# jagannatharjun/AntiZ

Measured on AMD Instinct MI355X. Metric: input MB/s precompressed (1 GB synthetic, 100k streams) at 1/2/4/8 MI355X, higher is better.
Workload: dtype u8

## Files before the change

antiz_amd/csrc/k_deflate.hip:

```cpp
#include <hip/hip_runtime.h>
#include "atz_device.h"

#define LDS __attribute__((address_space(3)))
#define CONSTANT __attribute__((address_space(4)))
#define GLOBAL __attribute__((address_space(1)))

#ifndef ATZ_VISITED_CHECK
#define ATZ_VISITED_CHECK 1
#endif
#ifndef ATZ_VISITED_MAX
#define ATZ_VISITED_MAX 8
#endif
#ifndef ATZ_NOSLIDE_PATH
#define ATZ_NOSLIDE_PATH 1
#endif
#ifndef ATZ_STEP_SPLIT
#define ATZ_STEP_SPLIT 0
#endif
#ifndef ATZ_STEP_CLOCKS
#define ATZ_STEP_CLOCKS 0
#endif
#if ATZ_STEP_CLOCKS
#define STEP_CLOCK() clock64()
#else
// ... 572 lines not shown
    o.x = (bf > 2 ? (bf << 23) | (df << 8) : 0u) | s0;
    if (jb.fast) o.y = ((p - reach) << 16) | (budget_out << 12) | (slot << 1) | valid;
    else o.y = (bq > 2 ? (bq << 23) | (dq << 8) : 0u) | valid;
    r[p] = o;
  }
}

__global__ __launch_bounds__(256) void k_match(const uint8_t* __restrict__ infl, const uint32_t* __restrict__ chains,
                                              uint2* __restrict__ R, const MatchJob* __restrict__ jobs) {
  const MatchJob jb = jobs[blockIdx.x];
  const uint8_t* in = infl + jb.infl_off;
  match_positions(jb, in, reinterpret_cast<const uint32_t*>(in), chains, R);
}

static constexpr uint32_t PREV_NIL = 0xffffu;
#ifndef ATZ_MATCH_THREADS
#define ATZ_MATCH_THREADS 1024
#endif
static constexpr uint32_t MATCH_THREADS = ATZ_MATCH_THREADS;
struct LdsWin {
  const LDS uint32_t* p;
  uint32_t off;
  __device__ __forceinline__ uint32_t operator[](uint32_t w) const { return p[w - off]; }
};
__global__ __launch_bounds__(MATCH_THREADS) void k_match_lds(const uint8_t* __restrict__ infl, const uint32_t* __restrict__ chains,
                                                  uint2* __restrict__ R, const MatchJob* __restrict__ jobs) {
  extern __shared__ uint32_t dyn_lds[];
  const MatchJob jb = jobs[blockIdx.x];
  const uint8_t* in = infl + jb.infl_off;
  const uint32_t* g32 = reinterpret_cast<const uint32_t*>(in);
  const uint32_t n = (uint32_t)jb.n, npad = (n + 63) & ~63u;
  const uint32_t* sidx = chains + jb.chain_off;
  const uint32_t* bpos = sidx + npad;
  const uint32_t maxdist = (1u << jb.window) - 262;
  const uint32_t lo = (uint32_t)jb.p0 > maxdist ? ((uint32_t)jb.p0 - maxdist) & ~3u : 0u;
  const uint32_t w0 = lo >> 2;
  const uint64_t want = jb.p1 + 258 + 24;
  const uint32_t nw = (uint32_t)(((want < n ? want : n) + 3) >> 2) - w0;
  LDS uint32_t* l32 = (LDS uint32_t*)dyn_lds;
  LDS uint16_t* prv = (LDS uint16_t*)(l32 + nw + 8);
  for (uint32_t w = threadIdx.x; w < nw + 8; w += MATCH_THREADS) l32[w] = w < nw ? g32[w0 + w] : 0u;
  const uint32_t nh = n >= 3 ? n - 2 : 0;
  const uint32_t P = (uint32_t)jb.p1 < nh ? (uint32_t)jb.p1 : nh;
  auto pred = [&](uint32_t a, uint32_t b) -> uint16_t {
    const uint32_t pq = b & ~BUCKET_FIRST;
    return ((a & BUCKET_FIRST) || pq < lo) ? (uint16_t)PREV_NIL : (uint16_t)(pq - lo);
  };
  if (P > lo && 4 * (P - lo) >= nh) {
    for (uint32_t i0 = 0; i0 < nh; i0 += 8 * MATCH_THREADS) {
      uint32_t a[8], b[8];
#pragma unroll
      for (int u = 0; u < 8; u++) {
        const uint32_t i = i0 + MATCH_THREADS * u + threadIdx.x;
        a[u] = i < nh ? bpos[i] : BUCKET_FIRST | 0x7fffffffu;
        b[u] = (i < nh && i) ? bpos[i - 1] : 0u;
      }
#pragma unroll
      for (int u = 0; u < 8; u++) {
        const uint32_t q = a[u] & ~BUCKET_FIRST;
        if (q >= lo && q < P) prv[q - lo] = pred(a[u], b[u]);
      }
    }
  } else {
    for (uint32_t q0 = lo; q0 < P; q0 += 8 * MATCH_THREADS) {
      uint32_t ix[8], a[8], b[8];
#pragma unroll
      for (int u = 0; u < 8; u++) { const uint32_t q = q0 + MATCH_THREADS * u + threadIdx.x; ix[u] = q < P ? sidx[q] : 1u; }
#pragma unroll
      for (int u = 0; u < 8; u++) { a[u] = bpos[ix[u]]; b[u] = ix[u] ? bpos[ix[u] - 1] : 0u; }
#pragma unroll
      for (int u = 0; u < 8; u++) {
        const uint32_t q = q0 + MATCH_THREADS * u + threadIdx.x;
        if (q < P) prv[q - lo] = pred(a[u], b[u]);
      }
    }
  }
  __syncthreads();
  const LdsWin in32{l32, w0};
  auto byte = [&](uint32_t x) -> uint32_t { return (in32[x >> 2] >> (8 * (x & 3))) & 0xffu; };
  uint2* r = R + jb.r_off;
  const uint32_t B = c_cfg[jb.level][3], nice = c_cfg[jb.level][2], Bq = B >> 2;
  const uint32_t hbits = jb.memlevel + 7u, hmask = (1u << hbits) - 1u, hshift = (hbits + 2u) / 3u;
  for (uint32_t p = (uint32_t)jb.p0 + threadIdx.x; p < (uint32_t)jb.p1; p += MATCH_THREADS) {
    uint32_t bf = 2, df = 0, bq = 2, dq = 0, valid = 0, slot = 0, budget_out = 0;
    uint32_t reach = p;
    const uint32_t s0 = byte(p);
    if (p + 3 <= n) {
      slot = (((s0 << (2 * hshift)) ^ (byte(p + 1) << hshift) ^ byte(p + 2)) & hmask) & (HOLE_SLOTS_M - 1);
      const uint32_t lim = p > maxdist ? p - maxdist : 0u;
      const uint32_t h0 = prv[p - lo];
      uint32_t cur = h0 + lo;
      if (h0 != PREV_NIL && cur >= 1 && cur + maxdist >= p) {
        valid = 1;
        const uint32_t left = n - p;
        const uint32_t cap = left < 258 ? left : 258u;
        const uint32_t nn = nice < cap ? nice : cap;
        uint32_t pv[4];
        load16(in32, p, pv);
        for (uint32_t i = 0;;) {
          reach = cur;
          const uint32_t nr = prv[cur - lo];
          const bool more = nr != PREV_NIL;
          const uint32_t nx = nr + lo;
          uint32_t len = match16(in32, cur, p, pv, 0);
          if (len == 16)
            while (len < cap) {
              const uint32_t l2 = match16(in32, cur + len, p + len, nullptr, 0);
              len += l2;
              if (l2 < 16) break;
            }
          if (len > cap) len = cap;
          if (len > bf) {
            bf = len; df = p - cur;
            if (i < Bq) { bq = len; dq = df; }
            if (len >= nn) break;
          }
          if (++i == B) {
            budget_out = (more && nx > lim) ? 1u : 0u;
            break;
          }
          if (!more) break;
          cur = nx;
          if (cur <= lim) break;
        }
      }
    }
    uint2 o;
    o.x = (bf > 2 ? (bf << 23) | (df << 8) : 0u) | s0;
    if (jb.fast) o.y = ((p - reach) << 16) | (budget_out << 12) | (slot << 1) | valid;
    else o.y = (bq > 2 ? (bq << 23) | (dq << 8) : 0u) | valid;
    r[p] = o;
  }
}

static constexpr int NLC = 286, NDC = 30, NBLC = 19, HEAPN = 2 * NLC + 1;
static constexpr uint32_t LOOKMIN = 262;
static constexpr uint32_t BITMAP_BITS = 32768;
static constexpr uint32_t HOLE_SLOTS = HOLE_SLOTS_M;

struct TreeWork {
  uint32_t heap[HEAPN + 1];
  uint16_t bl_count[16];
  uint32_t blc32[16];
};

struct TreeScratch {
  uint16_t anc[2][HEAPN];
  uint8_t dep[2][HEAPN];
  uint16_t freq[NLC];
};

struct BitOut {
  GLOBAL uint8_t* out;
  uint64_t cap;
  uint64_t pos;
  uint64_t bb;
  uint32_t bc;
  const GLOBAL uint8_t* orig;
  uint64_t clen;
  uint64_t shortcut;
  uint64_t eq_all;
  uint64_t eq_sc;
  int overflow;
  uint64_t cyc_tree, cyc_emit, blocks;
  uint64_t cyc_heap, cyc_scan, cyc_send;
};

static constexpr uint32_t STAGE_WORDS = 196;
struct BlockFreq {
  uint32_t lfreq2[(NLC + 1) / 2];
  uint32_t dfreq2[NDC / 2];
};
struct TreeCodes {
  uint16_t lcode[NLC]; uint8_t llen[NLC + 2];
  uint16_t dcode[NDC]; uint8_t dlen[NDC + 2];
  uint16_t bcode[NBLC]; uint8_t blen[NBLC + 2];
  uint32_t bfreq[NBLC];
  TreeWork w;
};
struct TrialShared {
  BitOut b;
  BlockFreq f;
  TreeCodes k;
  uint64_t stop_at;
  uint32_t stop_j, pad_;
};

template <uint32_t INS>
struct TrialSharedFast {
  static constexpr uint32_t INS_BITS = INS;
  TrialShared t;
  uint64_t ring[512];
  uint32_t ins[INS / 32];
  uint32_t holes[HOLE_SLOTS];
};

static constexpr uint32_t RING_SLOW = 512;
struct TrialSharedSlow {
  TrialShared t;
  uint64_t ring[RING_SLOW];
};
static_assert(sizeof(TreeScratch) <= RING_SLOW * sizeof(uint64_t), "tree scratch overlays the ring");
static_assert(offsetof(BitOut, cyc_scan) == offsetof(BitOut, cyc_heap) + 8, "block_trees' cyc[0], cyc[1]");
static_assert(STAGE_WORDS * 4 <= RING_SLOW * sizeof(uint64_t), "emission staging overlays the ring");

#ifndef ATZ_MW_F
#define ATZ_MW_F 3
#endif
static constexpr int MW_F = ATZ_MW_F;
struct MWSlot {
  BlockFreq f;
  int64_t block_start;
  uint64_t p, S;
  uint32_t last_lit, sbase, last, seq;
};
struct MWFlusher {
  TreeCodes k;
  TreeScratch sc;
  uint64_t cyc_tree, cyc_emit;
  uint64_t cyc_heap, cyc_scan;
};
static_assert(offsetof(MWFlusher, cyc_scan) == offsetof(MWFlusher, cyc_heap) + 8, "block_trees' cyc[0], cyc[1]");
struct MWCtl {
  uint32_t next_emit;
  uint32_t stop;
  uint32_t parse_done, nblocks;
  uint32_t state, hazard;
};
struct MWPart {
  MWSlot slot[MW_F];
  MWFlusher fl[MW_F];
  MWCtl ctl;
};
template <uint32_t INS>
struct TrialSharedFastMW {
  static constexpr uint32_t INS_BITS = INS;
  TrialShared t;
  uint64_t ring[512];
  uint32_t ins[INS / 32];
  uint32_t holes[HOLE_SLOTS];
  MWPart mw;
};
struct TrialSharedSlowMW {
  TrialShared t;
  uint64_t ring[RING_SLOW];
  MWPart mw;
};
static_assert(sizeof(TrialSharedFastMW<BITMAP_BITS>) <= 64 * 1024 && sizeof(TrialSharedSlowMW) <= 64 * 1024, "static LDS of a block");
template <typename T> struct HasMW { static constexpr bool value = false; };
template <uint32_t INS> struct HasMW<TrialSharedFastMW<INS>> { static constexpr bool value = true; };
template <> struct HasMW<TrialSharedSlowMW> { static constexpr bool value = true; };
__device__ __forceinline__ uint32_t ld_acq(const LDS uint32_t& x) {
  return uni(__hip_atomic_load(&x, __ATOMIC_ACQUIRE, __HIP_MEMORY_SCOPE_WORKGROUP));
}
__device__ __forceinline__ void st_rel(LDS uint32_t& x, uint32_t v, int lane) {
  if (lane == 0) __hip_atomic_store(&x, v, __ATOMIC_RELEASE, __HIP_MEMORY_SCOPE_WORKGROUP);
}

struct SweepArgs {
  const uint8_t* file;
  const uint8_t* infl;
  const uint32_t* chains;
  const uint2* R;
  const StreamDev* streams;
  const Trial* trials;
  TrialRes* res;
  uint32_t* stopj;
  uint8_t* out;
  uint32_t* syms;
  const uint32_t* adler;
  SweepOpts o;
  uint32_t ntrials;
};

__device__ inline uint64_t wsum64(uint64_t v) {
  for (int d = 32; d >= 1; d >>= 1) {
    uint32_t lo = __shfl_xor((uint32_t)v, d, 64), hi = __shfl_xor((uint32_t)(v >> 32), d, 64);
    v += ((uint64_t)hi << 32) | lo;
  }
  return v;
}

__device__ inline void emit_bytes_from_stage(LDS BitOut& b, const LDS uint32_t* stage, uint32_t nb, int lane) {
  uint32_t eqa = 0, eqs = 0;
  nb = uni(nb);
  const uint64_t pos = uni(b.pos), cap = uni(b.cap), clen = uni(b.clen), sc = uni(b.shortcut);
  GLOBAL uint8_t* const out = (GLOBAL uint8_t*)(uintptr_t)uni((uint64_t)(uintptr_t)b.out);
  const GLOBAL uint8_t* const orig = (const GLOBAL uint8_t*)(uintptr_t)uni((uint64_t)(uintptr_t)b.orig);
  for (uint32_t w = (uint32_t)lane; 4 * w < nb; w += 64) {
    const uint32_t word = stage[w];
#pragma unroll
    for (uint32_t j = 0; j < 4; j++) {
      const uint32_t k = 4 * w + j;
      const uint8_t x = (uint8_t)(word >> (8 * j));
      const uint64_t at = pos + k;
      if (k < nb && at < cap) out[at] = x;
      if (k < nb && at < clen) {
        const uint32_t e = orig[at] == x ? 1u : 0u;
        eqa += e;
        if (at < sc) eqs += e;
      }
    }
  }
  b.eq_all += wsum64(eqa);
  b.eq_sc += wsum64(eqs);
  if (pos + nb > cap) b.overflow = 1;
  b.pos = pos + nb;
}

__device__ inline void put_bits(LDS BitOut& b, LDS uint32_t* stage, uint32_t v, uint32_t n, int lane) {
  const uint32_t bc = uni(b.bc) + n;
  const uint64_t bb = uni(b.bb) | ((uint64_t)uni(v) << uni(b.bc));
  if (bc >= 32) {
    if (lane == 0) stage[0] = (uint32_t)bb;
    emit_bytes_from_stage(b, stage, 4, lane);
    b.bb = bb >> 32;
    b.bc = bc - 32;
  } else {
    b.bb = bb;
    b.bc = bc;
  }
}
__device__ inline void flush_bits_bytes(LDS BitOut& b, LDS uint32_t* stage, int lane) {
  const uint32_t bc = uni(b.bc), nb = bc >> 3;
  if (!nb) return;
  const uint64_t bb = uni(b.bb);
  if (lane == 0) { stage[0] = (uint32_t)bb; stage[1] = (uint32_t)(bb >> 32); }
  emit_bytes_from_stage(b, stage, nb, lane);
  b.bb = nb >= 8 ? 0 : (bb >> (8 * nb));
  b.bc = bc - 8 * nb;
}
__device__ inline void windup(LDS BitOut& b, LDS uint32_t* stage, int lane) {
  flush_bits_bytes(b, stage, lane);
  if (uni(b.bc)) {
    if (lane == 0) stage[0] = (uint32_t)b.bb;
    emit_bytes_from_stage(b, stage, 1, lane);
    b.bb = 0; b.bc = 0;
  }
}

__device__ __forceinline__ uint32_t tkey(uint32_t f, uint32_t d, uint32_t n) { return (f << 15) | (d << 10) | n; }

__device__ __forceinline__ void pq_down(LDS uint32_t* heap, int heap_len, int k, int lane) {
  const uint32_t v = uni(heap[k]);
  const uint32_t vk = v >> 10;
  const int t_l = 31 - __builtin_clz((uint32_t)lane + 2u);
  const int off_l = lane + 2 - (1 << t_l);
  for (;;) {
    if (2 * k > heap_len) break;
    const int idx = (k << t_l) + off_l;
    const uint32_t g = (t_l <= 5 && idx <= heap_len) ? heap[idx] : 0xffffffffu;
    int p = k;
    bool stop = false;
    int lj = 0;
#pragma unroll
    for (int t = 1; t <= 5; t++) {
      const uint32_t hl = (uint32_t)__builtin_amdgcn_readlane((int)g, lj);
      const uint32_t hr = (uint32_t)__builtin_amdgcn_readlane((int)g, lj + 1);
      const uint32_t c = (hr >> 10) <= (hl >> 10) ? 1u : 0u;
      const uint32_t hj = c ? hr : hl;
      if (vk <= (hj >> 10)) { stop = true; break; }
      heap[p] = hj;
      p = 2 * p + (int)c;
      lj = 2 * (lj + (int)c) + 2;
    }
    k = p;
    if (stop) break;
  }
  heap[k] = v;
}

template <typename T> __device__ __forceinline__ const CONSTANT T* uni_ptr(const CONSTANT T* p) {
  return (const CONSTANT T*)(uintptr_t)uni((uint64_t)(uintptr_t)p);
}
template <typename T> __device__ __forceinline__ const GLOBAL T* uni_ptr(const GLOBAL T* p) {
  return (const GLOBAL T*)(uintptr_t)uni((uint64_t)(uintptr_t)p);
}

struct TreeRes {
  int max_code;
  uint64_t d_opt, d_static;
};

__device__ __noinline__ TreeRes build_tree(LDS TreeWork& w, LDS TreeScratch& sc, LDS uint8_t* lenv, int elems, int max_length, const CONSTANT uint8_t* xbits,
                                           int xbase, const CONSTANT uint8_t* stlen, LDS uint64_t& cyc_heap, int lane) {
  elems = (int)uni((uint32_t)elems);
  max_length = (int)uni((uint32_t)max_length);
  xbase = (int)uni((uint32_t)xbase);
  xbits = uni_ptr(xbits);
  stlen = uni_ptr(stlen);
  uint64_t opt_len = 0, static_len = 0;
  const uint64_t lt = lane ? (~0ull >> (64 - lane)) : 0ull;
  LDS uint32_t* const heap = w.heap;
  int heap_len = 0, max_code = -1;
  for (int g = 0; g < elems; g += 64) {
    const int n = g + lane;
    const uint32_t f = n < elems ? sc.freq[n] : 0u;
    const uint64_t m = __ballot(f != 0);
    if (f) heap[heap_len + 1 + __popcll(m & lt)] = tkey(f, 0, (uint32_t)n);
    else if (n < elems) lenv[n] = 0;
    if (m) max_code = g + 63 - __clzll((long long)m);
    heap_len += __popcll(m);
  }
  while (heap_len < 2) {
    const int node = max_code < 2 ? ++max_code : 0;
    ++heap_len;
    if (lane == 0) { heap[heap_len] = tkey(1, 0, (uint32_t)node); sc.freq[node] = 1; }
    opt_len--;
    if (stlen) static_len -= stlen[node];
  }
  const uint64_t ch0 = STEP_CLOCK();
  int heap_max = HEAPN;
  uint32_t node = (uint32_t)elems;
  uint32_t root;
  if (heap_len <= 63) {
    uint32_t H = lane >= 1 && lane <= heap_len ? heap[lane] : 0xffffffffu;
    auto rd = [&](int i) -> uint32_t { return (uint32_t)__builtin_amdgcn_readlane((int)H, i); };
    auto wr = [&](int i, uint32_t v) { H = lane == i ? v : H; };
    auto down = [&](int len, int k) {
      const uint32_t v = rd(k), vk = v >> 10;
      int j = k << 1;
      bool go = j <= len;
      while (go) {
        const uint32_t a = rd(j), b = rd(j + 1);
        const uint32_t c = (b >> 10) <= (a >> 10) ? 1u : 0u;
        const uint32_t hj = c ? b : a;
        j += (int)c;
        go = vk > (hj >> 10);
        if (go) { wr(k, hj); k = j; j = k << 1; go = j <= len; }
      }
      wr(k, v);
    };
    for (int n = heap_len / 2; n >= 1; n--) down(heap_len, n);
    do {
      const uint32_t kn = rd(1);
      wr(1, rd(heap_len));
      wr(heap_len, 0xffffffffu);
      heap_len--;
      down(heap_len, 1);
      const uint32_t km = rd(1);
      const uint32_t dn = (kn >> 10) & 31u, dm = (km >> 10) & 31u;
      if (lane == 0) {
        heap[--heap_max] = kn & 1023u;
        heap[--heap_max] = km & 1023u;
        sc.anc[1][kn & 1023u] = (uint16_t)node;
        sc.anc[1][km & 1023u] = (uint16_t)node;
      } else {
        heap_max -= 2;
      }
      wr(1, tkey((kn >> 15) + (km >> 15), (dn >= dm ? dn : dm) + 1u, node));
      node++;
      down(heap_len, 1);
    } while (heap_len >= 2);
    root = rd(1) & 1023u;
  } else {
  for (int n = heap_len / 2; n >= 1; n--) pq_down(heap, heap_len, n, lane);
  do {
    const uint32_t kn = uni(heap[1]);
    heap[1] = uni(heap[heap_len]);
    heap_len--;
    pq_down(heap, heap_len, 1, lane);
    const uint32_t km = uni(heap[1]);
    const uint32_t dn = (kn >> 10) & 31u, dm = (km >> 10) & 31u;
    if (lane == 0) {
      heap[--heap_max] = kn & 1023u;
      heap[--heap_max] = km & 1023u;
      sc.anc[1][kn & 1023u] = (uint16_t)node;
      sc.anc[1][km & 1023u] = (uint16_t)node;
    } else {
      heap_max -= 2;
    }
    heap[1] = tkey((kn >> 15) + (km >> 15), (dn >= dm ? dn : dm) + 1u, node);
    node++;
    pq_down(heap, heap_len, 1, lane);
  } while (heap_len >= 2);
  root = uni(heap[1]) & 1023u;
  }
  if (lane == 0) cyc_heap += STEP_CLOCK() - ch0;
  --heap_max;
  if (lane == 0) heap[heap_max] = root;
  const int nn = (int)node;
  for (int i = lane; i < nn; i += 64) {
    const bool in_tree = i >= elems || (i <= max_code && sc.freq[i] != 0);
    const bool r = (uint32_t)i == root || !in_tree;
    sc.anc[0][i] = r ? (uint16_t)root : sc.anc[1][i];
    sc.dep[0][i] = r ? 0 : 1;
  }
  int cur = 0;
  for (int round = 0; round < 5; round++) {
    for (int i = lane; i < nn; i += 64) {
      const uint32_t a = sc.anc[cur][i];
      sc.dep[cur ^ 1][i] = (uint8_t)(sc.dep[cur][i] + sc.dep[cur][a]);
      sc.anc[cur ^ 1][i] = sc.anc[cur][a];
    }
    cur ^= 1;
  }
  if (lane < 16) w.blc32[lane] = 0;
  int overflow = 0;
  for (int g = 0; g < nn; g += 64) {
    const int i = g + lane;
    bool in_tree = false;
    uint32_t bits = 0;
    if (i < nn) {
      in_tree = i >= elems || (i <= max_code && sc.freq[i] != 0);
      bits = sc.dep[cur][i];
    }
    const bool capped = in_tree && (uint32_t)i != root && bits > (uint32_t)max_length;
    overflow += __popcll(__ballot(capped));
    if (bits > (uint32_t)max_length) bits = (uint32_t)max_length;
    const bool leaf = in_tree && i <= max_code;
    if (leaf) {
      lenv[i] = (uint8_t)bits;
      __hip_atomic_fetch_add(&w.blc32[bits], 1u, __ATOMIC_RELAXED, __HIP_MEMORY_SCOPE_WORKGROUP);
    }
  }
  uint32_t blc = lane >= 1 && lane < 16 ? w.blc32[lane] : 0u;
  if (overflow) {
    auto bl = [&](int b) -> uint32_t { return (uint32_t)__builtin_amdgcn_readlane((int)blc, b); };
    auto blset = [&](int b, uint32_t v) { blc = lane == b ? v : blc; };
    do {
      int bits = max_length - 1;
      while (bl(bits) == 0) bits--;
      blset(bits, bl(bits) - 1);
      blset(bits + 1, bl(bits + 1) + 2);
      blset(max_length, bl(max_length) - 1);
      overflow -= 2;
    } while (overflow > 0);
    int h = HEAPN;
    for (int bits = max_length; bits != 0; bits--) {
      uint32_t cnt = bl(bits);
      while (cnt != 0) {
        const uint32_t m = uni(heap[--h]);
        if ((int)m > max_code) continue;
        if (lane == 0) lenv[m] = (uint8_t)bits;
        cnt--;
      }
    }
  }
  if (lane < 16) w.bl_count[lane] = (uint16_t)blc;
  uint64_t o = 0, st = 0;
  for (int n = lane; n < elems && n <= max_code; n += 64) {
    const uint32_t f = sc.freq[n];
    if (f) {
      const uint32_t l = lenv[n];
      const uint32_t xb = (xbits && n >= xbase) ? xbits[n - xbase] : 0u;
      o += (uint64_t)f * (l + xb);
      if (stlen) st += (uint64_t)f * (stlen[n] + xb);
    }
  }
  opt_len += wsum64(o);
  if (stlen) static_len += wsum64(st);
  return TreeRes{max_code, opt_len, static_len};
}

__device__ __noinline__ void gen_codes(const LDS TreeWork& w, int max_code, LDS uint16_t* codes, LDS uint8_t* lens,
                                       int lane) {
  max_code = (int)uni((uint32_t)max_code);
  const bool lb = lane >= 1 && lane <= 15;
  const uint32_t bc = lb ? (uint32_t)w.bl_count[lane] : 0u;
  const uint32_t wv = bc << ((15 - lane) & 15);
  uint32_t nc = lb ? (wave_incl_scan(wv) - wv) >> (15 - lane) : 0u;
  const uint64_t lt = lane ? (~0ull >> (64 - lane)) : 0ull;
  const uint64_t present = __ballot(bc != 0);
  for (int g = 0; g <= max_code; g += 64) {
    const int n = g + lane;
    const uint32_t l = n <= max_code ? lens[n] : 0u;
    uint32_t mine = 0;
    for (uint64_t pm = present; pm; pm &= pm - 1) {
      const int b = __ffsll((unsigned long long)pm) - 1;
      const uint64_t m = __ballot(l == (uint32_t)b);
      if (!m) continue;
      const uint32_t base = (uint32_t)__builtin_amdgcn_readlane((int)nc, b);
      if (l == (uint32_t)b) mine = base + (uint32_t)__popcll(m & lt);
      if (lane == b) nc += (uint32_t)__popcll(m);
    }
    if (n <= max_code && l) codes[n] = (uint16_t)(__builtin_bitreverse32(mine) >> (32 - l));
  }
}

__device__ __forceinline__ uint32_t len_code(uint32_t len) {
  if (len < 8) return len;
  if (len == 255) return 28;
  const uint32_t lg = 31u - (uint32_t)__clz(len);
  return 4u * (lg - 1u) + ((len >> (lg - 2u)) & 3u);
}
__device__ __forceinline__ uint32_t dist_code(uint32_t d) {
  if (d < 4) return d;
  const uint32_t lg = 31u - (uint32_t)__clz(d);
  return 2u * lg + ((d >> (lg - 1u)) & 1u);
}
__device__ __forceinline__ uint32_t lcode_extra(uint32_t c) { return (c < 8 || c == 28) ? 0u : (c - 4) >> 2; }
__device__ __forceinline__ uint32_t lcode_base(uint32_t c) {
  return c < 8 ? c : c == 28 ? 255u : ((4 + (c & 3)) << lcode_extra(c));
}
__device__ __forceinline__ uint32_t dcode_extra(uint32_t d) { return d < 2 ? 0u : (d >> 1) - 1; }
__device__ __forceinline__ uint32_t dcode_base(uint32_t d) { return d < 2 ? d : ((2 + (d & 1)) << dcode_extra(d)); }


__device__ inline uint32_t early_exit(const LDS BitOut& b, const SweepOpts& o, uint64_t best_ident, bool full_needed) {
  if (uni((uint32_t)b.overflow)) return TR_OVERFLOW;
  if (full_needed) return ~0u;
  const uint64_t pos = uni(b.pos), clen = uni(b.clen), sc = uni(b.shortcut);
  if (sc) {
    uint64_t seen = pos < sc ? pos : sc;
    uint64_t mism = seen - uni(b.eq_sc);
    uint64_t thr = o.shortcut_len - o.recomp_tresh;
    if (thr > sc || mism > sc - thr) return TR_SHORTCUT;
  }
  if (pos > clen + o.sizediff_tresh) return TR_SIZEDIFF;
  uint64_t seen = pos < clen ? pos : clen;
  if (clen - (seen - uni(b.eq_all)) <= best_ident) return TR_CANT_BEAT;
  return ~0u;
}

static constexpr uint32_t SYM_PER_LANE = 2;
template <typename C16, typename C8>
__device__ __forceinline__ void sym_bits(uint32_t sy, bool valid, bool end, C16 lc, C8 ll, C16 dc, C8 dl,
                                         uint64_t& v, uint32_t& nb) {
  v = 0; nb = 0;
  if (valid) {
    uint32_t dist = sy >> 8;
    const uint32_t c = sy & 0xff;
    if (dist == 0) {
      v = lc[c]; nb = ll[c];
    } else {
      const uint32_t code = len_code(c);
      v = lc[code + 257]; nb = ll[code + 257];
      const uint32_t xe = lcode_extra(code);
      if (xe) { v |= (uint64_t)(c - lcode_base(code)) << nb; nb += xe; }
      dist--;
      const uint32_t dcd = dist_code(dist);
      v |= (uint64_t)dc[dcd] << nb; nb += dl[dcd];
      const uint32_t xd = dcode_extra(dcd);
      if (xd) { v |= (uint64_t)(dist - dcode_base(dcd)) << nb; nb += xd; }
    }
  } else if (end) {
    v = lc[256]; nb = ll[256];
  }
}
__device__ __forceinline__ void stage_or(LDS uint32_t* stage, uint32_t off, uint64_t v, uint32_t nb) {
  if (!nb) return;
  const uint32_t wi = off >> 5, sh = off & 31;
  const uint64_t lo = v << sh;
  const uint32_t hi = sh ? (uint32_t)(v >> (64 - sh)) : 0;
  __atomic_fetch_or(&stage[wi], (uint32_t)lo, __ATOMIC_RELAXED);
  if ((uint32_t)(lo >> 32)) __atomic_fetch_or(&stage[wi + 1], (uint32_t)(lo >> 32), __ATOMIC_RELAXED);
  if (hi) __atomic_fetch_or(&stage[wi + 2], hi, __ATOMIC_RELAXED);
}
__device__ uint32_t rle_tree(LDS TreeCodes& s, LDS uint32_t* stage, const LDS uint8_t* ln, int max_code, bool send,
                             uint32_t off, int lane) {
  const int N = max_code + 1;
  const int G = N / 64 + 1;
  uint64_t M[5];
#pragma unroll
  for (int g = 0; g < 5; g++) {
    M[g] = 0;
    if (g < G) {
      const int n = 64 * g + lane;
      bool st = false;
      if (n == 0 || n == N) st = true;
      else if (n < N) st = ln[n] != ln[n - 1];
      M[g] = __ballot(st);
    }
  }
  for (int g = 0; g < G; g++) {
    const int n = 64 * g + lane;
    uint64_t v64 = 0;
    uint32_t nb = 0;
    if (n < N) {
      int st = -1, en = -1;
      const uint64_t le = (lane == 63) ? ~0ull : ((2ull << lane) - 1);
#pragma unroll
      for (int h = 4; h >= 0; h--)
        if (st < 0 && h <= g) {
          const uint64_t m = h == g ? (M[h] & le) : M[h];
          if (m) st = 64 * h + 63 - __clzll((long long)m);
        }
#pragma unroll
      for (int h = 0; h < 5; h++)
        if (en < 0 && h >= g) {
          const uint64_t m = h == g ? (M[h] & ~le) : M[h];
          if (m) en = 64 * h + __ffsll((unsigned long long)m) - 1;
        }
      const uint32_t v = ln[n];
      const int k = n - st, R = en - st;
      int cnt = 0, minc = 3;
      bool first = false;
      if (v != 0) {
        if (k == 0) { cnt = R < 7 ? R : 7; minc = 4; first = true; }
        else if (k >= 7 && (k - 7) % 6 == 0) cnt = R - k < 6 ? R - k : 6;
      } else if (k % 138 == 0) {
        cnt = R - k < 138 ? R - k : 138;
      }
      if (cnt) {
        if (!send) {
          if (cnt < minc) __atomic_fetch_add(&s.bfreq[v], (uint32_t)cnt, __ATOMIC_RELAXED);
          else if (v != 0) {
            if (first) __atomic_fetch_add(&s.bfreq[v], 1u, __ATOMIC_RELAXED);
            __atomic_fetch_add(&s.bfreq[16], 1u, __ATOMIC_RELAXED);
          } else __atomic_fetch_add(&s.bfreq[cnt <= 10 ? 17 : 18], 1u, __ATOMIC_RELAXED);
        } else {
          const uint32_t cv = s.bcode[v], cl = s.blen[v];
          if (cnt < minc) {
            for (int q = 0; q < cnt; q++) { v64 |= (uint64_t)cv << nb; nb += cl; }
          } else if (v != 0) {
            if (first) { v64 = cv; nb = cl; }
            v64 |= (uint64_t)s.bcode[16] << nb; nb += s.blen[16];
            v64 |= (uint64_t)(cnt - (first ? 1 : 0) - 3) << nb; nb += 2;
          } else if (cnt <= 10) {
            v64 = s.bcode[17]; nb = s.blen[17];
            v64 |= (uint64_t)(cnt - 3) << nb; nb += 3;
          } else {
            v64 = s.bcode[18]; nb = s.blen[18];
            v64 |= (uint64_t)(cnt - 11) << nb; nb += 7;
          }
        }
      }
    }
    if (send) {
      const uint32_t incl = wave_incl_scan(nb);
      stage_or(stage, off + incl - nb, v64, nb);
      off += (uint32_t)__builtin_amdgcn_readlane((int)incl, 63);
    }
  }
  return off;
}

template <typename C16, typename C8>
__device__ bool compress_block(LDS BitOut& b, LDS uint32_t* stage, const GLOBAL uint32_t* syms, uint32_t nsym,
                               C16 lc, C8 ll, C16 dc, C8 dl, const SweepOpts& o, uint64_t best_ident,
                               bool full_needed, int lane) {
  __builtin_amdgcn_fence(__ATOMIC_ACQ_REL, "workgroup");
  for (uint32_t base = 0; base <= nsym; base += 64 * SYM_PER_LANE) {
    const uint32_t k0 = base + SYM_PER_LANE * (uint32_t)lane;
    const uint64_t sp = *(const GLOBAL uint64_t*)(syms + k0);
    uint64_t v0, v1;
    uint32_t n0, n1;
    sym_bits((uint32_t)sp, k0 < nsym, k0 == nsym, lc, ll, dc, dl, v0, n0);
    sym_bits((uint32_t)(sp >> 32), k0 + 1 < nsym, k0 + 1 == nsym, lc, ll, dc, dl, v1, n1);
    const uint32_t nb = n0 + n1;
    const uint32_t incl = wave_incl_scan(nb);
    const uint32_t total = (uint32_t)__builtin_amdgcn_readlane((int)incl, 63);
    if (total == 0) break;
    for (int i = lane; i < (int)STAGE_WORDS; i += 64) stage[i] = 0;
    const uint32_t bc = uni(b.bc);
    if (lane == 0) { stage[0] = (uint32_t)b.bb; stage[1] = (uint32_t)(b.bb >> 32); }
    const uint32_t off = bc + incl - nb;
    stage_or(stage, off, v0, n0);
    stage_or(stage, off + n0, v1, n1);
    const uint32_t all = bc + total;
    const uint32_t full = all >> 3;
    emit_bytes_from_stage(b, stage, full, lane);
    const uint32_t rem = all & 7;
    const uint32_t lastw = stage[full >> 2];
    b.bb = rem ? ((lastw >> (8 * (full & 3))) & 0xff) & ((1u << rem) - 1) : 0;
    b.bc = rem;
    if (!full_needed && early_exit(b, o, best_ident, false) != ~0u) return true;
  }
  return false;
}

struct Lz {
  uint32_t level, kind, wsize, maxdist, lbs, good, lazy, nice, chain;
  uint32_t n;
  uint32_t p;
  uint32_t lookahead;
  uint32_t S;
  uint32_t block_start;
  uint32_t match_start, prev_match;
  uint32_t match_length, prev_length;
  int match_available;
  uint32_t last_lit;
  uint32_t nsym;
};

__device__ __forceinline__ void fill(Lz& z) {
  do {
    uint32_t sw = z.p - z.S;
    uint32_t more = 2u * z.wsize - z.lookahead - sw;
    if (sw >= z.wsize + z.maxdist) { z.S += z.wsize; more += z.wsize; }
    uint32_t rd = z.p + z.lookahead;
    if (rd >= z.n) break;
    uint32_t k = z.n - rd;
    if (k > more) k = more;
    z.lookahead += k;
  } while (z.lookahead < LOOKMIN && z.p + z.lookahead < z.n);
}

__device__ inline uint32_t common_len(const uint8_t* in, uint64_t a, uint64_t b, uint32_t from, uint32_t cap,
                                      int lane) {
  for (uint32_t k0 = from; k0 < cap; k0 += 64) {
    uint32_t k = k0 + lane;
    bool ne = k < cap && in[a + k] != in[b + k];
    if (k >= cap) ne = true;
    uint64_t m = __ballot(ne);
    if (m) {
      uint32_t f = k0 + (uint32_t)(__ffsll((unsigned long long)m) - 1);
      return f < cap ? f : cap;
    }
  }
  return cap;
}

struct BlockPlan {
  uint64_t opt_lenb, static_lenb;
  int lmax, dmax, max_blindex;
};
__device__ __noinline__ BlockPlan block_trees(const LDS BlockFreq& f, LDS TreeCodes& s, LDS TreeScratch& sc, LDS uint64_t* cyc,
                                              uint32_t level, uint64_t stored_len, int lane) {
  level = uni(level);
  stored_len = uni(stored_len);
  BlockPlan pl{};
  uint64_t opt_len = 0, static_len = 0;
  if (level > 0) {
    for (int i = lane; i < NLC; i += 64) sc.freq[i] = (uint16_t)(f.lfreq2[i >> 1] >> (16 * (i & 1)));
    TreeRes r = build_tree(s.w, sc, s.llen, NLC, 15, (const CONSTANT uint8_t*)c_xlb, 257, (const CONSTANT uint8_t*)c_t.st_llen,
                           cyc[0], lane);
    pl.lmax = (int)uni((uint32_t)r.max_code);
    opt_len += uni(r.d_opt);
    static_len += uni(r.d_static);
    gen_codes(s.w, pl.lmax, s.lcode, s.llen, lane);
    for (int i = pl.lmax + 1 + lane; i < NLC + 2; i += 64) s.llen[i] = 0;
    for (int i = lane; i < NDC; i += 64) sc.freq[i] = (uint16_t)(f.dfreq2[i >> 1] >> (16 * (i & 1)));
    r = build_tree(s.w, sc, s.dlen, NDC, 15, (const CONSTANT uint8_t*)c_xdb, 0, (const CONSTANT uint8_t*)c_t.st_dlen,
                   cyc[0], lane);
    pl.dmax = (int)uni((uint32_t)r.max_code);
    opt_len += uni(r.d_opt);
    static_len += uni(r.d_static);
    gen_codes(s.w, pl.dmax, s.dcode, s.dlen, lane);
    for (int i = pl.dmax + 1 + lane; i < NDC + 2; i += 64) s.dlen[i] = 0;
    for (int i = lane; i < NBLC; i += 64) s.bfreq[i] = 0;
    const uint64_t cs0 = STEP_CLOCK();
    rle_tree(s, nullptr, s.llen, pl.lmax, false, 0, lane);
    rle_tree(s, nullptr, s.dlen, pl.dmax, false, 0, lane);
    if (lane == 0) cyc[1] += STEP_CLOCK() - cs0;
    for (int i = lane; i < NBLC; i += 64) sc.freq[i] = (uint16_t)s.bfreq[i];
    r = build_tree(s.w, sc, s.blen, NBLC, 7, (const CONSTANT uint8_t*)c_xblb, 0, nullptr, cyc[0], lane);
    const int bmax = (int)uni((uint32_t)r.max_code);
    opt_len += uni(r.d_opt);
    gen_codes(s.w, bmax, s.bcode, s.blen, lane);
    for (int i = bmax + 1 + lane; i < NBLC + 2; i += 64) s.blen[i] = 0;
    int mb;
    for (mb = NBLC - 1; mb >= 3; mb--)
      if (s.blen[bl_order((uint32_t)mb)] != 0) break;
    pl.max_blindex = mb;
    opt_len += 3 * ((uint64_t)mb + 1) + 5 + 5 + 4;
    pl.opt_lenb = (opt_len + 3 + 7) >> 3;
    pl.static_lenb = (static_len + 3 + 7) >> 3;
    if (pl.static_lenb <= pl.opt_lenb) pl.opt_lenb = pl.static_lenb;
  } else {
    pl.opt_lenb = pl.static_lenb = stored_len + 5;
  }
  return pl;
}

__device__ __noinline__ uint32_t block_emit(LDS TreeCodes& s, LDS uint32_t* stage, LDS BitOut& b, const GLOBAL uint32_t* syms,
                                            const GLOBAL uint8_t* in, int64_t block_start, uint64_t p, uint64_t S,
                                            uint32_t last_lit, uint32_t lbs, int last, SweepOpts opt, uint64_t best_ident,
                                            bool full_needed, uint64_t opt_lenb, uint64_t static_lenb, int lmax, int dmax,
                                            int max_blindex, int lane) {
  syms = uni_ptr(syms);
  in = uni_ptr(in);
  block_start = (int64_t)uni((uint64_t)block_start);
  p = uni(p);
  S = uni(S);
  last_lit = uni(last_lit);
  lbs = uni(lbs);
  last = (int)uni((uint32_t)last);
  opt.recomp_tresh = uni(opt.recomp_tresh);
  opt.sizediff_tresh = uni(opt.sizediff_tresh);
  opt.shortcut_len = uni(opt.shortcut_len);
  opt.mismatch_tol = uni(opt.mismatch_tol);
  best_ident = uni(best_ident);
  full_needed = uni((uint32_t)full_needed) != 0;
  opt_lenb = uni(opt_lenb);
  static_lenb = uni(static_lenb);
  lmax = (int)uni((uint32_t)lmax);
  dmax = (int)uni((uint32_t)dmax);
  max_blindex = (int)uni((uint32_t)max_blindex);
  uint32_t hazard = 0;
  const bool bufok = block_start >= (int64_t)S;
  const uint64_t stored_len = (uint64_t)((int64_t)p - block_start);
  const uint64_t blk_start_bytes = b.pos;
  b.blocks++;
  if (stored_len + 4 <= opt_lenb && bufok) {
    put_bits(b, stage, (uint32_t)last, 3, lane);
    windup(b, stage, lane);
    uint32_t len = (uint32_t)stored_len;
    put_bits(b, stage, (len & 0xffff) | ((~len & 0xffff) << 16), 32, lane);
    const GLOBAL uint8_t* src = in + block_start;
    for (uint64_t o = 0; o < stored_len; o += 256) {
      uint32_t nb = stored_len - o < 256 ? (uint32_t)(stored_len - o) : 256u;
      for (uint32_t k = lane; k < 64; k += 64) {
        uint32_t wv = 0;
        for (int q = 0; q < 4; q++) {
          uint32_t at = 4 * k + q;
          if (at < nb) wv |= (uint32_t)src[o + at] << (8 * q);
        }
        stage[k] = wv;
      }
      emit_bytes_from_stage(b, stage, nb, lane);
      if (!full_needed && early_exit(b, opt, best_ident, false) != ~0u) break;
    }
  } else if (static_lenb == opt_lenb) {
    const uint32_t bc0 = uni(b.bc);
    b.bb = uni(b.bb) | ((uint64_t)((1u << 1) + (uint32_t)last) << bc0);
    b.bc = bc0 + 3;
    compress_block(b, stage, syms, last_lit, (const CONSTANT uint16_t*)c_t.st_lcode, (const CONSTANT uint8_t*)c_t.st_llen,
                   (const CONSTANT uint16_t*)c_t.st_dcode, (const CONSTANT uint8_t*)c_t.st_dlen, opt, best_ident,
                   full_needed, lane);
  } else {
    int lcodes = lmax + 1, dcodes = dmax + 1, blcodes = max_blindex + 1;
    const uint64_t cs0 = STEP_CLOCK();
    for (int i = lane; i < (int)STAGE_WORDS; i += 64) stage[i] = 0;
    const uint32_t bc0 = uni(b.bc);
    const uint64_t bb0 = uni(b.bb);
    if (lane == 0) { stage[0] = (uint32_t)bb0; stage[1] = (uint32_t)(bb0 >> 32); }
    uint32_t off = bc0;
    if (lane == 0)
      stage_or(stage, off, (uint64_t)((2u << 1) + (uint32_t)last) | ((uint64_t)(lcodes - 257) << 3) |
                               ((uint64_t)(dcodes - 1) << 8) | ((uint64_t)(blcodes - 4) << 13), 17);
    off += 17;
    if (lane < blcodes) stage_or(stage, off + 3u * (uint32_t)lane, s.blen[bl_order((uint32_t)lane)], 3);
    off += 3u * (uint32_t)blcodes;
    off = rle_tree(s, stage, s.llen, lcodes - 1, true, off, lane);
    off = rle_tree(s, stage, s.dlen, dcodes - 1, true, off, lane);
    {
      const uint32_t full = off >> 3;
      emit_bytes_from_stage(b, stage, full, lane);
      const uint32_t rem = off & 7;
      const uint32_t lastw = stage[full >> 2];
      b.bb = rem ? ((lastw >> (8 * (full & 3))) & 0xff) & ((1u << rem) - 1) : 0;
      b.bc = rem;
    }
    b.cyc_send += STEP_CLOCK() - cs0;
    compress_block(b, stage, syms, last_lit, (const LDS uint16_t*)s.lcode, (const LDS uint8_t*)s.llen,
                   (const LDS uint16_t*)s.dcode, (const LDS uint8_t*)s.dlen, opt, best_ident, full_needed, lane);
  }
  if (b.pos - blk_start_bytes > (uint64_t)lbs + 2ull * last_lit && last_lit) hazard = 1;
  if (last) windup(b, stage, lane);
  return hazard;
}

__device__ __forceinline__ void init_block(LDS BlockFreq& f, int lane) {
  for (int i = lane; i < (NLC + 1) / 2; i += 64) f.lfreq2[i] = 0;
  for (int i = lane; i < NDC / 2; i += 64) f.dfreq2[i] = 0;
  if (lane == 0) f.lfreq2[128] = 1;
}

__device__ __forceinline__ uint32_t flush_block(LDS TrialShared& s, LDS TreeScratch& sc, LDS BitOut& b, const GLOBAL uint32_t* syms,
                                                const GLOBAL uint8_t* in, int64_t block_start, uint64_t p, uint64_t S,
                                                uint32_t last_lit, uint32_t level, uint32_t lbs, int last, const SweepOpts& opt,
                                                uint64_t best_ident, bool full_needed, int lane) {
  const uint64_t c0 = clock64();
  const BlockPlan pl = block_trees(s.f, s.k, sc, &b.cyc_heap, level, (uint64_t)((int64_t)p - block_start), lane);
  const uint64_t c1 = clock64();
  b.cyc_tree += c1 - c0;
  const uint32_t hz = block_emit(s.k, (LDS uint32_t*)&sc, b, syms, in, block_start, p, S, last_lit, lbs, last, opt, best_ident,
                                 full_needed, pl.opt_lenb, pl.static_lenb, pl.lmax, pl.dmax, pl.max_blindex, lane);
  init_block(s.f, lane);
  b.cyc_emit += clock64() - c1;
  return hz;
}

struct WinPath {
  uint64_t H;
  uint32_t end;
  bool need;
};
__device__ __forceinline__ uint32_t run_end_rel(uint64_t Am, int lane) {
  const uint64_t above = lane == 63 ? 0ull : (Am >> (lane + 1));
  return (uint32_t)lane + 1u + (uint32_t)__builtin_ctzll(~above);
}
__device__ __forceinline__ WinPath follow_path(uint32_t rel, uint64_t Nm, uint32_t lim) {
  WinPath w;
  uint64_t H = 0;
  uint32_t i = 0;
  while (i < lim) {
    H |= 1ull << i;
    i = (uint32_t)__builtin_amdgcn_readlane((int)rel, (int)i);
  }
  w.need = (H & Nm) != 0;
  if (w.need) {
    i = 63u - (uint32_t)__builtin_clzll(H & Nm);
    H &= ~Nm;
  }
  w.H = H;
  w.end = i;
  return w;
}
__device__ __forceinline__ void path_lane(const WinPath& w, uint64_t Am, uint32_t ma_in, int lane, bool& onp,
                                          uint32_t& mab) {
  const uint64_t le = lane == 63 ? ~0ull : ((2ull << lane) - 1ull);
  const uint64_t hb = w.H & le;
  onp = false;
  mab = 0;
  if (hb) {
    const int h = 63 - __builtin_clzll(hb);
    if (h == lane) {
      onp = true;
      const uint64_t hs = w.H & (le >> 1);
      mab = hs ? (uint32_t)((Am >> (63 - __builtin_clzll(hs))) & 1ull) : ma_in;
    } else if ((Am >> h) & 1ull) {
      const uint64_t seg = le & ~((1ull << h) - 1ull);
      onp = (~Am & seg) == 0;
      mab = 1;
    }
  }
}
__device__ __forceinline__ uint32_t wave_excl_sum(uint32_t cnt, uint64_t lt, uint32_t& total) {
  uint32_t o = 0, T = 0;
  for (uint32_t bit = 0; bit < 32; bit++) {
    const uint64_t m = __ballot((cnt >> bit) & 1u);
    o += (uint32_t)__popcll(m & lt) << bit;
    T += (uint32_t)__popcll(m) << bit;
    if (!__ballot(cnt >> (bit + 1))) break;
  }
  total = T;
  return o;
}

__device__ __forceinline__ void spec_init(LDS TrialShared& s, const SweepArgs& A, const Trial& tr, int lane) {
  if (lane == 0) {
    s.stop_at = A.stopj ? (uint64_t)(uintptr_t)(A.stopj + tr.stream) : 0ull;
    s.stop_j = tr.spec_j;
  }
}
__device__ __forceinline__ bool spec_stopped(const LDS TrialShared& s) {
  const uint64_t a = uni(s.stop_at);
  const uint32_t j = uni(s.stop_j);
  if (!a || !j) return false;
  return uni(__hip_atomic_load((const GLOBAL uint32_t*)(uintptr_t)a, __ATOMIC_RELAXED, __HIP_MEMORY_SCOPE_AGENT)) < j;
}
__device__ __forceinline__ void spec_stop(const LDS TrialShared& s, const SweepArgs& A, uint64_t best_ident, uint32_t state,
                                          uint64_t ident, uint64_t clen, int lane) {
  const uint64_t a = uni(s.stop_at);
  if (!a || state != TR_FULL || ident <= best_ident) return;
  if (ident != clen && ident + A.o.mismatch_tol < clen) return;
  if (lane == 0) __hip_atomic_fetch_min((GLOBAL uint32_t*)(uintptr_t)a, uni(s.stop_j), __ATOMIC_RELAXED, __HIP_MEMORY_SCOPE_AGENT);
}

__device__ void trial_flusher(const SweepArgs& A, LDS TrialShared& s, LDS MWPart& mw, const Trial& tr,
                              const GLOBAL uint32_t* syms, const GLOBAL uint8_t* in, uint32_t level, uint32_t lbs,
                              bool full_needed, int f, int lane) {
  LDS BitOut& b = s.b;
  LDS MWFlusher& me = mw.fl[f];
  LDS MWSlot& sl = mw.slot[f];
  LDS MWCtl& ctl = mw.ctl;
// ... 956 lines not shown
```

Measured before the change: 1693.

## Parallelize heap sift-down across wave lanes and trim stage zeroing

Replaces the serial readlane-based sift-down from the root of the small Huffman heap with a wave-parallel version. It uses DPP sibling comparison, ballots to find the min-child path, bpermute to shift path elements up, and a ballot to locate the landing slot. It also merges the two wave sums for equality counts into one packed scan, and zeroes only the stage words the current batch can touch instead of the whole buffer. The aim is to cut serial per-step cross-lane latency in tree building and bit emission. The trade-off is tricky bit logic: the packed 16-bit counters could overflow and the path mask could be computed wrongly.

```diff
diff --git a/antiz_amd/csrc/k_deflate.hip b/antiz_amd/csrc/k_deflate.hip
--- a/antiz_amd/csrc/k_deflate.hip
+++ b/antiz_amd/csrc/k_deflate.hip
@@ -898,8 +898,9 @@
       }
     }
   }
-  b.eq_all += wsum64(eqa);
-  b.eq_sc += wsum64(eqs);
+  const uint32_t eq2 = (uint32_t)__builtin_amdgcn_readlane((int)wave_incl_scan(eqa | (eqs << 16)), 63);
+  b.eq_all += eq2 & 0xffffu;
+  b.eq_sc += eq2 >> 16;
   if (pos + nb > cap) b.overflow = 1;
   b.pos = pos + nb;
 }
@@ -1027,13 +1028,29 @@
       }
       wr(k, v);
     };
+    const uint32_t l1 = (uint32_t)lane >> 1, l2 = (uint32_t)lane >> 2, l3 = (uint32_t)lane >> 3, l4 = (uint32_t)lane >> 4;
+    const uint32_t odd = (uint32_t)lane & 1u, nz = lane ? 1u : 0u;
+    auto down_root = [&](int len, uint32_t v) {
+      const uint32_t K = H >> 10, vk = v >> 10;
+      const uint32_t N = (uint32_t)__builtin_amdgcn_update_dpp(0, (int)K, 0xB1, 0xf, 0xf, false);
+      const uint64_t M = __ballot(K < N + odd);
+      const uint32_t cb = lane < 32 ? (uint32_t)(M >> (2 * lane + 1)) & 1u : 0u;
+      const uint32_t G = (uint32_t)__builtin_amdgcn_ds_bpermute((int)(((2u * (uint32_t)lane + cb) & 63u) << 2), (int)H);
+      const uint64_t C = M | 3ull;
+      const uint32_t Cl = (uint32_t)C;
+      const uint32_t on = (uint32_t)(C >> lane) & (Cl >> l1) & (Cl >> l2) & (Cl >> l3) & (Cl >> l4) & nz;
+      const uint64_t P = __ballot(on != 0) & ((2ull << len) - 1ull);
+      const uint64_t hit = __ballot(vk <= K) & P & ~2ull;
+      const int land = hit ? (__builtin_ctzll(hit) >> 1) : 63 - __builtin_clzll(P);
+      H = on != 0 && lane < land ? G : (lane == land ? v : H);
+    };
     for (int n = heap_len / 2; n >= 1; n--) down(heap_len, n);
     do {
       const uint32_t kn = rd(1);
-      wr(1, rd(heap_len));
+      const uint32_t vl = rd(heap_len);
       wr(heap_len, 0xffffffffu);
       heap_len--;
-      down(heap_len, 1);
+      down_root(heap_len, vl);
       const uint32_t km = rd(1);
       const uint32_t dn = (kn >> 10) & 31u, dm = (km >> 10) & 31u;
       if (lane == 0) {
@@ -1044,9 +1061,8 @@
       } else {
         heap_max -= 2;
       }
-      wr(1, tkey((kn >> 15) + (km >> 15), (dn >= dm ? dn : dm) + 1u, node));
+      down_root(heap_len, tkey((kn >> 15) + (km >> 15), (dn >= dm ? dn : dm) + 1u, node));
       node++;
-      down(heap_len, 1);
     } while (heap_len >= 2);
     root = rd(1) & 1023u;
   } else {
@@ -1338,8 +1354,9 @@
     const uint32_t incl = wave_incl_scan(nb);
     const uint32_t total = (uint32_t)__builtin_amdgcn_readlane((int)incl, 63);
     if (total == 0) break;
-    for (int i = lane; i < (int)STAGE_WORDS; i += 64) stage[i] = 0;
     const uint32_t bc = uni(b.bc);
+    const uint32_t nz = min((bc + total + 31u) / 32u + 2u, STAGE_WORDS);
+    for (uint32_t i = (uint32_t)lane; i < nz; i += 64) stage[i] = 0;
     if (lane == 0) { stage[0] = (uint32_t)b.bb; stage[1] = (uint32_t)(b.bb >> 32); }
     const uint32_t off = bc + incl - nb;
     stage_or(stage, off, v0, n0);
```

Measured after the change: 1735, median of 3. 2.5% higher.
